# vaibhawvipul/taper

Hardware: AMD Instinct MI355X
Metric: MNIST samples/sec fwd+bwd+step (higher is better)
Workload: dtype f32; 1 GPU; mlp_784-128-10_b64; per_gpu_batch=64, global_batch=64, parallelism=single, comm=none, graph_record_steps=11577

## Files before the change

### include/taper_hip.h

```cpp
#ifndef TAPER_HIP_H
#define TAPER_HIP_H

#include <stddef.h>
#include <stdint.h>

#ifdef __cplusplus
extern "C" {
#endif

typedef struct th_ctx th_ctx;
typedef struct th_graph th_graph;
typedef struct th_event th_event;
typedef struct th_comm th_comm;

typedef struct th_adam_fuse {
    float *d_p, *d_m, *d_v;
    const int32_t *d_t;
    const float *d_lr;
    float beta1, beta2, eps, weight_decay;
} th_adam_fuse;

typedef struct th_adam_slice {
    const float *d_g;
    int64_t n;
// ... 68 lines not shown
                               int64_t *d_state, int64_t advance, int32_t *d_adam_tick, const th_adam_fuse *w_fuse,
                               const th_adam_fuse *b_fuse, int mask_dh_by_h);

int th_linear_xent_wide(th_ctx *ctx, const float *d_x, const float *d_w, const float *d_bias, const float *d_targets,
                        int batch, int in_features, int classes, float *d_loss, float *d_ncorrect,
                        float *d_dx, float *d_dw, float *d_db, float *d_metrics, int64_t metrics_capacity,
                        int64_t *d_state, int64_t advance, int32_t *d_adam_tick);
int th_linear_xent_wide_ex(th_ctx *ctx, const float *d_x, const float *d_w, const float *d_bias, const float *d_targets, int batch,
                           int in_features, int classes, float *d_loss, float *d_ncorrect, float *d_dx, float *d_dw, float *d_db,
                           float *d_metrics, int64_t metrics_capacity, int64_t *d_state, int64_t advance, int32_t *d_adam_tick,
                           float *d_colsum_masked);
int th_bias_from_colsum_adam(th_ctx *ctx, const float *d_colsum, float *d_gb, int c, int hw, const th_adam_fuse *b_fuse,
                             const th_adam_slice *extra, int n_extra);
typedef struct th_wide_fuse {
    th_adam_fuse w, b, conv_b;
    float *d_conv_gb;
    int conv_c, conv_hw;
} th_wide_fuse;
int th_linear_xent_wide_fused(th_ctx *ctx, const float *d_x, const float *d_w, const float *d_bias, const float *d_targets, int batch,
                              int in_features, int classes, float *d_loss, float *d_ncorrect, float *d_dw, float *d_db,
                              float *d_metrics, int64_t metrics_capacity, int64_t *d_state, int64_t advance, int32_t *d_adam_tick,
                              float *d_colsum_masked, const th_wide_fuse *fuse);

int th_mlp_tail_supported(int batch, int in_features, int hidden, int classes, int need_dx);
int th_mlp_tail(th_ctx *ctx, const float *d_x, const float *d_h, const float *d_w2, const float *d_b2,
                const float *d_targets, int batch, int in_features, int hidden, int classes,
                float *d_loss, float *d_ncorrect, float *d_dw1, float *d_db1, float *d_dw2, float *d_db2,
                const float *d_w1, float *d_dx,
                float *d_metrics, int64_t metrics_capacity, int64_t *d_state, int64_t advance,
                const th_adam_fuse *w1_fuse, const th_adam_fuse *b1_fuse);

typedef struct th_mlp3_layer {
    const float *d_w, *d_b;
    float *d_dw, *d_db;
    const th_adam_fuse *w_fuse, *b_fuse;
    int out_features;
} th_mlp3_layer;
typedef struct th_mlp3_gap {
    const float *d_cnt;
    float *d_gb;
    int hw;
    const th_adam_fuse *b_fuse;
} th_mlp3_gap;
int th_mlp3_supported(int batch, int in_features, int h1, int h2, int classes);
int th_mlp3_xent(th_ctx *ctx, const float *d_x, const float *d_targets, int batch, int in_features, const th_mlp3_layer *layers,
                 float *d_dx, float *d_loss, float *d_ncorrect, float *d_metrics, int64_t metrics_capacity, int64_t *d_state,
// ... 285 lines not shown
```

### taper_amd/csrc/host/modules.cpp

```cpp
#include <algorithm>
#include <chrono>
#include <cmath>
#include <cstdio>
#include <cstdlib>
#include <cstring>
#include <fstream>

#include "nn_internal.h"

namespace taper {
static float *n_correct_slot(Tensor *n_correct_out) {
    if (!n_correct_out) return nullptr;
    *n_correct_out = Tensor::empty({1});
    return n_correct_out->dptr();
}

static float *grad_slot(const Tensor &p) {
    if (!p.defined()) return nullptr;
    if (!p.grad_->buf) p.grad_->buf = Buffer::alloc(p.len());
    p.grad_->known_zero = false;
    return p.grad_->buf->d;
}

Tensor log_softmax(const Tensor &x, int dim) {
// ... 225 lines not shown
    TAPER_ASSERT(mlp_tail_supported(x, w1, b1, w2, b2), "mlp_tail_cross_entropy: unsupported shapes / gradient state");
    TAPER_ASSERT(targets.shape()[0] == x.shape()[0], "Batch sizes must match");
    const int b = (int)x.shape()[0], in_f = (int)x.shape()[1], hid = (int)w1.shape()[0], c = (int)w2.shape()[0];
    th_ctx *ctx = Device::ctx();
    Adam *fa = FusedAdamScope::active();
    th_adam_slice carried[TH_MAX_ADAM_SLICES];
    const int n_carried = fa ? fa->take_deferred(w1.dptr(), carried) : 0;
    if (fa && fa->has_deferred()) fa->flush_deferred();
    Tensor h = Tensor::empty({(size_t)b, (size_t)hid});
    TH(th_linear_fwd_ex(ctx, x.dptr(), w1.dptr(), b1.defined() ? b1.dptr() : nullptr, h.dptr(), b, in_f, hid, 1, carried, n_carried,
                        fa ? fa->d_tick() : nullptr));
    Tensor loss = Tensor::empty({1});
    float *nc = n_correct_slot(n_correct_out);
    float *dw1 = grad_slot(w1), *db1 = grad_slot(b1), *dw2 = grad_slot(w2), *db2 = grad_slot(b2);
    const bool need_dx = x.get_requires_grad();
    std::shared_ptr<Buffer> dx = need_dx ? Buffer::alloc(x.len()) : nullptr;
    th_adam_fuse wf{}, bf{};
    const th_adam_fuse *pw = nullptr, *pb = nullptr;
    if (fa) {
        if (!need_dx && fa->fuse_for(w1, &wf)) pw = &wf;
        if (b1.defined() && fa->fuse_for(b1, &bf)) pb = &bf;
    }
    const Communicator *xc = log ? log->exchange : nullptr;
    if (xc && xc->n_ranks > 1) {
        TAPER_ASSERT(fa && !need_dx && xc->tail_exchange_ok(b, in_f, hid, c), "mlp_tail_cross_entropy: the in-launch exchange does not cover this step");
        TH(th_mlp_tail_dp(xc->handle(), ctx, x.dptr(), h.dptr(), w2.dptr(), b2.defined() ? b2.dptr() : nullptr, targets.dptr(), b, in_f, hid, c,
                          loss.dptr(), nc, dw1, db1, dw2, db2, log ? log->d_metrics : nullptr, log ? log->capacity : 0,
                          log ? log->d_state : nullptr, log ? log->advance : 0, pw, pb, fa->d_tick()));
    } else
    TH(th_mlp_tail(ctx, x.dptr(), h.dptr(), w2.dptr(), b2.defined() ? b2.dptr() : nullptr, targets.dptr(), b, in_f, hid, c, loss.dptr(),
                   nc, dw1, db1, dw2, db2, need_dx ? w1.dptr() : nullptr, dx ? dx->d : nullptr, log ? log->d_metrics : nullptr,
                   log ? log->capacity : 0, log ? log->d_state : nullptr, log ? log->advance : 0, pw, pb));
    if (fa) {
        if (need_dx) fa->defer_for(w1);
        fa->defer_for(w2);
        if (b2.defined()) fa->defer_for(b2);
    }
    loss.set_requires_grad(true);
    Tensor p1 = w1, p2 = b1, p3 = w2, p4 = b2, out = loss, keep = h, xin = x;
    Tape::push(loss, true, [p1, p2, p3, p4, out, keep, xin, dx]() {
        if (!out.has_grad()) return;
        TAPER_ASSERT(out.grad_->shared_const, "mlp_tail_cross_entropy: only loss.backward() from the root is supported");
        if (dx) {
            TAPER_ASSERT(!xin.has_grad() && !xin.grad_->buf_is_arena, "mlp_tail_cross_entropy: input already has a gradient");
            xin.grad_->buf = dx;
            xin.grad_->has = true;
// ... 397 lines not shown
```

### taper_amd/csrc/host/taper.h

```cpp
#pragma once

#include <algorithm>
#include <cstdint>
#include <functional>
#include <map>
#include <memory>
#include <random>
#include <stdexcept>
#include <string>
#include <vector>

#include "../../../include/taper_hip.h"

namespace taper {

struct Error : std::runtime_error {
    explicit Error(const std::string &m) : std::runtime_error(m) {}
};
void th_check(int rc, const char *what);
#define TAPER_ASSERT(cond, msg)                       \
    do {                                              \
        if (!(cond)) throw ::taper::Error(msg);       \
    } while (0)

// ... 576 lines not shown
    bool step_reduced(const class Communicator &comm);
    void set_step_guard(const uint32_t *d_error_word) { step_guard_ = d_error_word; }
    void zero_grad() override { fp_.zero_grad(); }
    float get_lr() const { return lr_; }
    void set_lr(float lr);
    float weight_decay() const { return wd_; }
    float beta1() const { return beta1_; }
    float beta2() const { return beta2_; }
    float eps() const { return eps_; }
    void set_weight_decay(float wd) { wd_ = wd; }
    void load_state(int t, const std::vector<float> &m, const std::vector<float> &v);
    int t() const;
    std::vector<float> m() const;
    std::vector<float> v() const;
    FlatParams &flat() override { return fp_; }

    int32_t *d_tick() const { return reinterpret_cast<int32_t *>(state_->d); }
    bool fuse_for(const Tensor &param, th_adam_fuse *out);
    bool fuse_for_slot(const std::shared_ptr<GradSlot> &slot, th_adam_fuse *out);
    bool defer_for(const Tensor &param);
    int take_deferred(const float *launch_reads, th_adam_slice *out);
    void flush_deferred();
    void set_carry_deferred(bool on) { carry_deferred_ = on; }
    bool has_deferred() const { return !deferred_.empty(); }
    bool step_open() const { for (char f : fused_) if (f) return true; return !deferred_.empty(); }
    void set_external_tick(bool on) { external_tick_ = on; }
    void drop_step_bookkeeping() { deferred_.clear(); std::fill(fused_.begin(), fused_.end(), 0); }

   private:
    FlatParams fp_;
    std::shared_ptr<Buffer> m_, v_, state_;
    float lr_, beta1_, beta2_, eps_, wd_;
    bool external_tick_ = false;
    bool carry_deferred_ = false;
    const uint32_t *step_guard_ = nullptr;
    std::vector<char> fused_;
    std::vector<th_adam_slice> deferred_;
};

class AdamW : public Optimizer {
   public:
    AdamW(const std::vector<Tensor> &params, float lr, float beta1 = 0.9f, float beta2 = 0.999f, float eps = 1e-8f,
          float weight_decay = 0.0f)
        : adam(params, lr, beta1, beta2, eps, weight_decay) {}
    void step() override;
    void zero_grad() override { adam.zero_grad(); }
    FlatParams &flat() override { return adam.flat(); }
    float get_lr() const { return adam.get_lr(); }
    void set_lr(float lr) { adam.set_lr(lr); }
    Adam adam;
};

class LRScheduler {
   public:
    virtual ~LRScheduler() = default;
    virtual void step(const float *metric ) = 0;
    virtual float get_lr() const = 0;
// ... 226 lines not shown
```

### taper_amd/csrc/host/trainer.cpp

```cpp
#include <algorithm>
#include <chrono>
#include <cmath>
#include <cstdio>
#include <cstdlib>
#include <cstring>
#include <fstream>

#include "nn_internal.h"
#include "../../../include/taper_hip_debug.h"

namespace taper {
MNISTDataset MNISTDataset::from_host(const std::vector<float> &images, const std::vector<float> &labels, bool train) {
    TAPER_ASSERT(images.size() == labels.size() * 784, "MNISTDataset: images must be [N,784]");
    MNISTDataset d;
    d.images = Tensor(images, {labels.size(), 784});
    d.labels = Tensor(labels, {labels.size()});
    d.train = train;
    return d;
}

MNISTDataset MNISTDataset::from_u8(const std::vector<uint8_t> &pixels, const std::vector<uint8_t> &labels, bool train) {
    TAPER_ASSERT(pixels.size() == labels.size() * 784, "MNISTDataset: pixels must be [N,784]");
    th_ctx *ctx = Device::ctx();
    MNISTDataset d;
// ... 332 lines not shown
        case StepForm::Mlp2Rows: {
            std::vector<Tensor> w, b;
            for (Linear *l : plan.linear)
                if (l) {
                    w.push_back(l->weight);
                    b.push_back(l->bias);
                }
            loss = mlp2_cross_entropy(*rows, batch, w, b, &ncorrect, &sink);
            break;
        }
        case StepForm::ChainMlp3:
        case StepForm::Mlp3: {
            const Tensor w3[3] = {L[0]->weight, L[1]->weight, L[2]->weight}, b3[3] = {L[0]->bias, L[1]->bias, L[2]->bias};
            loss = plan.form == StepForm::ChainMlp3 ? conv_chain_mlp3_cross_entropy(xin, plan.stages, w3, b3, y, &ncorrect, &sink)
                                                    : mlp3_cross_entropy(seq->forward_prefix(xin, plan.prefix), w3, b3, y, &ncorrect, &sink);
            break;
        }
        case StepForm::ChainHead:
            loss = conv_chain_head_cross_entropy(xin, plan.stages, L[0]->weight, L[0]->bias, y, &ncorrect, &sink);
            break;
        case StepForm::MlpTail: {
            Tensor xh = seq->forward_prefix(xin, plan.prefix);
            if (plan.fused_adam) adam->set_carry_deferred(true);
            loss = mlp_tail_cross_entropy(xh, L[0]->weight, L[0]->bias, L[1]->weight, L[1]->bias, y, &ncorrect, &sink);
            break;
        }
        case StepForm::LinearHead:
        case StepForm::LinearWide: {
            adam->flush_deferred();
            Tensor h = seq->forward_prefix(xin, plan.prefix);
            loss = plan.form == StepForm::LinearHead ? linear_cross_entropy(h, L[0]->weight, L[0]->bias, y, &ncorrect, &sink)
                                                     : linear_cross_entropy_wide(h, L[0]->weight, L[0]->bias, y, &ncorrect, &sink);
            break;
        }
        case StepForm::Layered: {
            adam->flush_deferred();
            qat_pass_.run(*model);
            Tensor h = seq ? seq->forward_prefix(xin, plan.prefix) : model->forward(xin);
            for (size_t i = plan.prefix; seq && i < seq->layers.size(); ++i) h = seq->layers[i]->forward(h);
            loss = cross_entropy_loss(h, y, &ncorrect, &sink);
            break;
        }
    }
    loss.backward();
    if (plan.exchange) {
        optimizer->step();
    } else if (!(comm && optimizer->step_reduced(*comm))) {
        reduce_grads(*this);
        optimizer->step();
        optimizer->set_step_guard(nullptr);
    }
    optimizer->zero_grad();
    adam->set_carry_deferred(false);
}

void Trainer::enqueue_steps(const float *d_images, const float *d_labels, const int32_t *d_indices, int64_t n_indices,
                            size_t batch, size_t steps) {
    int64_t *state = reinterpret_cast<int64_t *>(state_->d);
    struct Guard {
        Guard(const uint32_t *w, uint32_t *step) { TH(th_ctx_set_update_guard(Device::ctx(), w, step)); }
        ~Guard() { th_ctx_set_update_guard(Device::ctx(), nullptr, nullptr); }
    } guard(comm && comm->is_p2p() ? comm->error_word() : nullptr, comm && comm->is_p2p() ? comm->step_word() : nullptr);
    TH(th_linear_fwd_ex_set_subtiles(Device::ctx(), !(comm && comm->ranks_on_this_device() > 1)));
    const StepPlan plan = plan_step(batch, d_indices ? n_indices : (int64_t)batch);
    if (plan.form == StepForm::Mlp2Rows) {
        const th_row_source rows{d_images, d_labels, d_indices, d_indices ? state + 1 : nullptr, d_indices ? n_indices : 0,
                                 d_indices ? n_indices : (int64_t)batch};
        for (size_t s = 0; s < steps; ++s) enqueue_compute(plan, nullptr, nullptr, batch, &rows);
    } else if (d_indices == nullptr) {
        enqueue_compute(plan, const_cast<float *>(d_images), const_cast<float *>(d_labels), batch);
    } else {
        TH(th_gather_batch(Device::ctx(), d_images, d_labels, d_indices, n_indices, state + 1, (int)(batch * steps), 784, xb_->d,
                           yb_->d));
        for (size_t s = 0; s < steps; ++s) enqueue_compute(plan, xb_->d + s * batch * 784, yb_->d + s * batch, batch);
    }
    optimizer->flush_deferred();
// ... 135 lines not shown
        }
        std::sort(graphs_.begin(), graphs_.end(), [](const auto &x, const auto &y) { return x.first > y.first; });
        graph_key_ = key;
    }
    if (!whole) {
        const size_t tail = n_full - done > 0 ? (n_full - done) % chunk : 0;
        size_t exact = 0;
        for (auto &g : graphs_) exact += (g.first & (g.first - 1)) != 0 ? 1 : 0;
        if (tail > 2 && (tail & (tail - 1)) != 0 && !have(tail) && have(1) && exact < 4 && !graph_capture_failed_ &&
            graph_key_ == key) {
            TH(th_graph_begin(ctx));
            th_graph *g = nullptr;
            try {
                enqueue_steps(d_img, d_lab, d_idx, (int64_t)n, bs, tail);
                TH(th_graph_end(ctx, &g));
                graphs_.emplace_back(tail, g);
                std::sort(graphs_.begin(), graphs_.end(), [](const auto &x, const auto &y) { return x.first > y.first; });
            } catch (const std::exception &e) {
                fprintf(stderr, "taper: capturing a %zu-step remainder graph failed (%s); the ladder graphs serve it\n", tail, e.what());
                if (!g) th_graph_end(ctx, &g);
                if (g) th_graph_destroy(g);
                if (auto *adam = dynamic_cast<Adam *>(optimizer.get())) {
                    adam->set_carry_deferred(false);
                    adam->drop_step_bookkeeping();
                }
                optimizer->zero_grad();
                Tape::reset();
                if (!comm) throw;
            }
        }
    }
    if (!whole && done == 0 && nb == n_full && n_full >= 2 && have(n_full) && whole_graphs_.size() < 4 && !graph_capture_failed_ && graph_key_ == key &&
        std::find(whole_capture_failed_.begin(), whole_capture_failed_.end(), n_full) == whole_capture_failed_.end()) {
        TH(th_graph_begin(ctx));
        th_graph *g = nullptr;
        try {
            TH(th_fill_f32(ctx, state_->d, 0.f, 4));
            enqueue_steps(d_img, d_lab, d_idx, (int64_t)n, bs, n_full);
            TH(th_graph_end(ctx, &g));
            whole_graphs_.emplace_back(n_full, g);
            TH(th_graph_launch(ctx, g));
            done = n_full;
        } catch (const std::exception &e) {
            fprintf(stderr, "taper: capturing a whole-call graph of %zu steps failed (%s); reset + replay stay two launches\n", n_full, e.what());
            whole_capture_failed_.push_back(n_full);
            if (!g) th_graph_end(ctx, &g);
            if (g) th_graph_destroy(g);
            if (auto *adam = dynamic_cast<Adam *>(optimizer.get())) {
                adam->set_carry_deferred(false);
                adam->drop_step_bookkeeping();
            }
            optimizer->zero_grad();
            Tape::reset();
            if (!comm) throw;
        }
    }
    while (done < n_full) {
        bool launched = false;
        for (auto &g : graphs_) {
            if (done + g.first <= n_full) {
                TH(th_graph_launch(ctx, g.second));
                done += g.first;
                launched = true;
                break;
            }
        }
        if (!launched) {
            enqueue_steps(d_img, d_lab, d_idx, (int64_t)n, bs, 1);
            ++done;
        }
    }
    if (nb > n_full) {
// ... 32 lines not shown
```

### taper_amd/csrc/mlp_tail.hip

```cpp
#include "tail_dev.h"
#include "dp_dev.h"

TH_USES_DEVICE_ERRORS()

namespace th {

struct TailArgs {
    const float *x, *h, *w2, *b2, *targets;
    int batch, in_f, hid, c;
    float *loss, *ncorrect, *dw1, *db1, *dw2, *db2;
    float *metrics;
    int64_t capacity;
    int64_t *state;
    int64_t advance;
    AdamDev w1_adam, b1_adam;
    int n_dw, n_head, tiles_m, groups;
    const float *w1;
    float *dx;
    int xgroups;
    DpDev dp;
    int32_t *dp_tick;
};

#ifdef TH_PROFILE
// ... 416 lines not shown
    int64_t log_slot = 0, state0_next = 0, state1_next = 0;
    if (log) {
        const int64_t state0 = sload(a.state), state1 = sload(a.state + 1);
        log_slot = tail_log_slot(state0, a.capacity);
        state0_next = state0 + 1;
        state1_next = state1 + a.advance;
    }
    if (lane == 0) *h_step = step;
    __syncthreads();
    if (lead) {
        if (a.db2 && lane < a.c) {
            float sum = sc[0][16 + lane];
#pragma unroll
            for (int w = 1; w < NW; ++w) sum += sc[w][16 + lane];
            a.db2[lane] = sum;
        }
        if (lane == 0) tail_lead_log<NW>(a, sc, log_slot, state0_next, state1_next);
#ifdef TH_PROFILE
        if (lane == 0) tail_prof_end(wall_clock64());
#endif
    }
}

template <int KS, int TN, bool HAS_DX, int NW, int DPNR = 0>
__global__ __launch_bounds__(64 * (NW + tail_helper_waves(KS, NW, DPNR))) void mlp_tail_exact_kernel(TailArgs a) {
    constexpr unsigned HID = 16 * KS;
    constexpr bool HELPER = tail_helper_waves(KS, NW, DPNR) != 0;
    __shared__ float h_step;
    __shared__ float red[NW][TN][64][4];
    __shared__ float tr[NW][16][17];
    __shared__ float rowv[NW][2][16];
    __shared__ float sc[NW][36];
    asm volatile("" ::"s"(a.x), "s"(a.h), "s"(a.w2), "s"(a.b2), "s"(a.targets), "s"(a.batch), "s"(a.in_f), "s"(a.c), "s"(a.dw1),
                 "s"(a.db1), "s"(a.w1_adam.p), "s"(a.w1_adam.m), "s"(a.w1_adam.v), "s"(a.w1_adam.t), "s"(a.w1_adam.lr),
                 "s"(a.b1_adam.p), "s"(a.b1_adam.t), "s"(a.b1_adam.lr), "s"(a.n_dw), "s"(a.n_head), "s"(a.groups), "s"(a.metrics),
                 "s"(a.state));
    const int t = threadIdx.x, lane = t & 63, wave = t >> 6, r16 = lane & 15, g4 = lane >> 4;
    const int bid = blockIdx.x;
    TAIL_STAMP(0);
    DpTicket dp_tk{0u, 0u};
    if constexpr (DPNR > 0) dp_tk = dp_begin(a.dp);
    if (HAS_DX && bid >= a.n_head + a.n_dw) {
        if (!HELPER || wave < NW) tail_dx_role<KS, NW>(a, bid - a.n_head - a.n_dw);
        return;
    }
    const bool head_role = bid < a.n_head;
    int tile_m, grp = 0, tt = 0;
    if (!head_role) {
        const int b2 = bid - a.n_head;
        tt = (b2 & 7) * (a.n_dw >> 3) + (b2 >> 3);
        if (tt >= KS * a.groups) return;
        tile_m = tt % KS;
        grp = tt / KS;
    } else {
// ... 9 lines not shown
    if constexpr (HELPER) {
        if (__builtin_amdgcn_readfirstlane(wave) == NW) {
            tail_helper_wave<NW>(a, head_role, lead, any_w, any_b, &h_step, sc);
            return;
        }
    }
    const int32_t w_t = (!HELPER && any_w) ? sload(a.w1_adam.t) : 1, b_t = (!HELPER && any_b) ? sload(a.b1_adam.t) : 1;
    const float w_lr = (!HELPER && any_w) ? sload(a.w1_adam.lr) : 0.f, b_lr = (!HELPER && any_b) ? sload(a.b1_adam.lr) : 0.f;

    float4 wv[KS];
    const unsigned w_off = ((unsigned)min(r16, C - 1) * HID + g4 * 4) * 4u;
#pragma unroll
    for (int ks = 0; ks < KS; ++ks) wv[ks] = ldg4_b(a.w2, w_off + ks * 64);
    float w2b[4], b2v[4];
#pragma unroll
    for (int s = 0; s < 4; ++s) {
        const unsigned cls = (unsigned)min(g4 * 4 + s, C - 1);
        w2b[s] = ldg_b(a.w2, (cls * HID + hcol) * 4u);
        b2v[s] = a.b2 ? ldg_b(a.b2, cls * 4u) : 0.f;
    }
    bool tn_ok[TN];
#pragma unroll
    for (int tn = 0; tn < TN; ++tn) tn_ok[tn] = col0 + tn * 16 < in_f;
    const unsigned e_off = ((tile_m * 16 + g4 * 4 + wave) * in_f + col0 + r16) * 4u;
    const bool fuse_w = !head_role && any_w;
    const bool finisher = NW == 4 || wave < 4;
    float e_p[TN], e_m[TN], e_v[TN], w_step = 0.f, b_step = 0.f;
#pragma unroll
    for (int tn = 0; tn < TN; ++tn) {
        e_p[tn] = e_m[tn] = e_v[tn] = 0.f;
        if (fuse_w && tn_ok[tn] && finisher) {
            e_p[tn] = ldg_b(a.w1_adam.p, e_off + tn * 64);
            e_m[tn] = ldg_b(a.w1_adam.m, e_off + tn * 64);
            e_v[tn] = ldg_b(a.w1_adam.v, e_off + tn * 64);
        }
    }
    const bool fuse_b1 = head_role && any_b;
    const unsigned b1_off = (tile_m * 16 + (t & 15)) * 4u;
    float bp_ = 0.f, bm_ = 0.f, bv_ = 0.f;
    if (fuse_b1) {
        bp_ = ldg_b(a.b1_adam.p, b1_off);
        bm_ = ldg_b(a.b1_adam.m, b1_off);
        bv_ = ldg_b(a.b1_adam.v, b1_off);
    }
    const bool log_here = !HELPER && lead && a.metrics;
    const int64_t state0 = log_here ? sload(a.state) : 0, state1 = log_here ? sload(a.state + 1) : 0;

    floatx4 accdw[TN];
#pragma unroll
    for (int tn = 0; tn < TN; ++tn) accdw[tn] = floatx4{0.f, 0.f, 0.f, 0.f};
    floatx4 acc_dw2 = {0.f, 0.f, 0.f, 0.f};
    float db1_acc = 0.f, db2_acc = 0.f, nll_acc = 0.f, hit_acc = 0.f;
    const float inv_b = 1.0f / (float)B;

    float4 hv[KS];
    float tf = 0.f, hm[4], xv[TN][4];
    auto load_chunk = [&](int c0) {
        const int r0 = c0 + wave * 16;
        if (r0 >= B) return;
        const unsigned h_off = ((unsigned)(r0 + r16) * HID + g4 * 4) * 4u;
#pragma unroll
        for (int ks = 0; ks < KS; ++ks) hv[ks] = ldg4_b(a.h, h_off + ks * 64);
        tf = ldg_b(a.targets, (unsigned)(r0 + r16) * 4u);
        const unsigned hm_off = ((unsigned)(r0 + g4 * 4) * HID + hcol) * 4u;
        const unsigned x_off = ((unsigned)(r0 + g4 * 4) * in_f + col0 + r16) * 4u;
#pragma unroll
        for (int s = 0; s < 4; ++s) {
            hm[s] = ldg_b(a.h, hm_off + s * HID * 4);
#pragma unroll
            for (int tn = 0; tn < TN; ++tn)
                xv[tn][s] = (!head_role && tn_ok[tn]) ? ldg_b(a.x, x_off + s * in_f * 4u + tn * 64) : 0.f;
        }
    };
    load_chunk(0);
    TAIL_STAMP(1);
    if (!HELPER && fuse_w) w_step = adam_step_size(w_lr, a.w1_adam.beta1, a.w1_adam.beta2, w_t);
    if (!HELPER && fuse_b1) b_step = adam_step_size(b_lr, a.b1_adam.beta1, a.b1_adam.beta2, b_t);
    int64_t log_slot = 0, state0_next = 0, state1_next = 0;
    if (log_here) {
        log_slot = tail_log_slot(state0, a.capacity);
        state0_next = state0 + 1;
        state1_next = state1 + a.advance;
    }
    TAIL_STAMP(2);

    for (int c0 = 0;;) {
        const int r0 = c0 + wave * 16;
        const bool rows_here = r0 < B;
        if (rows_here) {
            TAIL_STAMP(3);
            floatx4 ax = {0.f, 0.f, 0.f, 0.f}, ay = ax, az = ax, aw = ax;
#pragma unroll
            for (int ks = 0; ks < KS; ++ks) {
                ax = __builtin_amdgcn_mfma_f32_16x16x4f32(wv[ks].x, hv[ks].x, ax, 0, 0, 0);
// ... 7 lines not shown
            for (int i = 0; i < 4; ++i) lg[i] = (g4 * 4 + i < C) ? ((ax[i] + ay[i]) + (az[i] + aw[i])) + b2v[i] : -INFINITY;
            tail_row_softmax(lg, g4, C, tf, inv_b, dl, nll_row, bi);
            TAIL_STAMP(4);

            floatx4 dh = {0.f, 0.f, 0.f, 0.f};
#pragma unroll
            for (int s = 0; s < 4; ++s) dh = __builtin_amdgcn_mfma_f32_16x16x4f32(dl[s], w2b[s], dh, 0, 0, 0);
            float dhm[4];
#pragma unroll
            for (int i = 0; i < 4; ++i) dhm[i] = hm[i] > 0.f ? dh[i] : 0.f;

            if (!head_role) {
#pragma unroll
                for (int s = 0; s < 4; ++s)
#pragma unroll
                    for (int tn = 0; tn < TN; ++tn)
                        accdw[tn] = __builtin_amdgcn_mfma_f32_16x16x4f32(dhm[s], xv[tn][s], accdw[tn], 0, 0, 0);
            } else {
                db1_acc += sum_over_g4((dhm[0] + dhm[1]) + (dhm[2] + dhm[3]));
                __builtin_amdgcn_wave_barrier();
#pragma unroll
                for (int i = 0; i < 4; ++i) tr[wave][r16][g4 * 4 + i] = dl[i];
                if (lead && g4 == 0) {
                    rowv[wave][0][r16] = nll_row;
                    rowv[wave][1][r16] = (fabsf((float)bi - tf) < 1e-6f) ? 1.f : 0.f;
                }
                __builtin_amdgcn_wave_barrier();
#pragma unroll
                for (int s = 0; s < 4; ++s)
                    acc_dw2 = __builtin_amdgcn_mfma_f32_16x16x4f32(tr[wave][g4 * 4 + s][r16], hm[s], acc_dw2, 0, 0, 0);
                if (lead) {
                    float cs = 0.f, nl = 0.f, ht = 0.f;
#pragma unroll
                    for (int r = 0; r < 16; ++r) {
                        cs += tr[wave][r][r16];
                        nl += rowv[wave][0][r];
                        ht += rowv[wave][1][r];
                    }
                    db2_acc += cs;
                    nll_acc += nl;
                    hit_acc += ht;
                }
            }
        }
        c0 += 16 * NW;
        if (c0 >= B) break;
        load_chunk(c0);
    }

    TAIL_STAMP(5);
    if (!head_role) {
#pragma unroll
        for (int tn = 0; tn < TN; ++tn)
#pragma unroll
            for (int i = 0; i < 4; ++i) red[wave][tn][lane][i] = accdw[tn][i];
        __syncthreads();
        TAIL_STAMP(6);
        if (HELPER && fuse_w) w_step = h_step;
        float outv[TN];
#pragma unroll
        for (int tn = 0; tn < TN; ++tn) {
            outv[tn] = 0.f;
            if (!tn_ok[tn] || !finisher) continue;
            float out = red[0][tn][lane][wave];
#pragma unroll
            for (int w = 1; w < NW; ++w) out += red[w][tn][lane][wave];
            outv[tn] = out;
        }
        if constexpr (DPNR > 0) {
            if (!dp_reduce<DPNR, TN>(a.dp, dp_tk, KS + tt, finisher ? t : -1, outv)) return;
        }
#pragma unroll
        for (int tn = 0; tn < TN; ++tn) {
            if (!tn_ok[tn] || !finisher) continue;
            const float out = outv[tn];
            if (DPNR == 0 || !fuse_w) *reinterpret_cast<float *>(reinterpret_cast<char *>(a.dw1) + e_off + tn * 64) = out;
            if (fuse_w) {
                const AdamDev &ad = a.w1_adam;
                const float gv = out + ad.wd * e_p[tn];
                const float mn = ad.beta1 * e_m[tn] + (1.0f - ad.beta1) * gv;
                const float vn = ad.beta2 * e_v[tn] + (1.0f - ad.beta2) * gv * gv;
                *reinterpret_cast<float *>(reinterpret_cast<char *>(ad.m) + e_off + tn * 64) = mn;
                *reinterpret_cast<float *>(reinterpret_cast<char *>(ad.v) + e_off + tn * 64) = vn;
                *reinterpret_cast<float *>(reinterpret_cast<char *>(ad.p) + e_off + tn * 64) = e_p[tn] - w_step * mn / (sqrtf(vn) + ad.eps);
            }
        }
        TAIL_STAMP(7);
        return;
    }

#pragma unroll
    for (int i = 0; i < 4; ++i) red[wave][0][lane][i] = acc_dw2[i];
    if (g4 == 0) sc[wave][r16] = db1_acc;
    if (lead && g4 == 0) sc[wave][16 + r16] = db2_acc;
    if (lead && lane == 0) {
        sc[wave][32] = nll_acc;
        sc[wave][33] = hit_acc;
    }
    __syncthreads();
    TAIL_STAMP(6);
    if (HELPER && fuse_b1) b_step = h_step;
    if constexpr (DPNR > 0) {
        float hv2[2] = {0.f, 0.f};
        const int cls = g4 * 4 + wave;
        if (a.dw2 && wave < 4 && cls < C) {
            float sum = red[0][0][lane][wave];
#pragma unroll
            for (int w = 1; w < NW; ++w) sum += red[w][0][lane][wave];
            hv2[0] = sum;
        }
        if (a.db1 && t < 16) {
            float out = sc[0][t];
#pragma unroll
            for (int w = 1; w < NW; ++w) out += sc[w][t];
            hv2[1] = out;
        } else if (lead && a.db2 && t >= 16 && t < 16 + C) {
            float sum = sc[0][t];
#pragma unroll
// ... 61 lines not shown
            }
            const float l = n / (float)B;
            a.loss[0] = l;
            if (a.ncorrect) a.ncorrect[0] = hsum;
            if (a.metrics) {
                a.metrics[2 * log_slot] = l;
                a.metrics[2 * log_slot + 1] = hsum;
                a.state[0] = state0_next;
                a.state[1] = state1_next;
            }
        }
    }
    TAIL_STAMP(7);
}

}

using namespace th;

static bool tail_whole_tiles(int batch, int in_features, int hidden) {
    return (hidden == 32 || hidden == 64 || hidden == 128 || hidden == 256) && batch % 16 == 0 && in_features % 16 == 0;
}

extern "C" int th_mlp_tail_supported(int batch, int in_features, int hidden, int classes, int need_dx) {
    const bool ok = batch > 0 && batch <= 512 && in_features > 0 && hidden > 0 && hidden <= 256 && (hidden % 4) == 0 && classes > 0 &&
                    classes <= 16;
    return ok && (!need_dx || tail_whole_tiles(batch, in_features, hidden));
}

static bool tail_dp_shapes(int batch, int in_features, int hidden, int classes) {
    return th_mlp_tail_supported(batch, in_features, hidden, classes, 0) && tail_whole_tiles(batch, in_features, hidden) &&
           (hidden == 64 || hidden == 128);
}
static int tail_dp_grid(int in_features, int hidden) {
    const int tiles_m = hidden / 16, groups = ceil_div(in_features, 32);
    return ((tiles_m * groups + 7) & ~7) + ((tiles_m + 7) & ~7);
}
template <int KS, int NW>
static const void *tail_dp_instance(int n_ranks) {
    if (n_ranks <= 2) return (const void *)mlp_tail_exact_kernel<KS, 2, false, NW, 2>;
    if (n_ranks <= 4) return (const void *)mlp_tail_exact_kernel<KS, 2, false, NW, 4>;
    return (const void *)mlp_tail_exact_kernel<KS, 2, false, NW, 8>;
}
static int tail_exact_threads(int ks, int nw, bool dp) { return 64 * (nw + tail_helper_waves(ks, nw, dp ? 2 : 0)); }
static const void *tail_dp_kernel(int batch, int hidden, int n_ranks) {
    const bool nw8 = batch > 64;
// ... 2 lines not shown
}

extern "C" int th_mlp_tail_dp_supported(const th_comm *comm, th_ctx *ctx, int batch, int in_features, int hidden, int classes) {
    const DpDev *dp = comm_dp_dev(comm);
    if (!dp || !ctx || dp->n_ranks < 2 || !tail_dp_shapes(batch, in_features, hidden, classes)) return 0;
    const int grid = tail_dp_grid(in_features, hidden);
    if (grid > DP_MAX_SLOTS) return 0;
    if (comm_dp_sharing(comm) > 1) {
        int per_cu = 0;
        if (hipOccupancyMaxActiveBlocksPerMultiprocessor(&per_cu, tail_dp_kernel(batch, hidden, dp->n_ranks), tail_exact_threads(hidden / 16, batch > 64 ? 8 : 4, true), 0) != hipSuccess) {
            (void)hipGetLastError();
            return 0;
        }
        if (!comm_dp_shared_fits(comm, grid, per_cu)) return 0;
    }
    return 1;
}

static int mlp_tail_launch(th_comm *comm, th_ctx *ctx, const float *d_x, const float *d_h, const float *d_w2, const float *d_b2,
                           const float *d_targets, int batch, int in_features, int hidden, int classes, float *d_loss,
                           float *d_ncorrect, float *d_dw1, float *d_db1, float *d_dw2, float *d_db2, const float *d_w1, float *d_dx,
                           float *d_metrics, int64_t metrics_capacity, int64_t *d_state, int64_t advance,
                           const th_adam_fuse *w1_fuse, const th_adam_fuse *b1_fuse, int32_t *d_tick) {
    TH_REQUIRE(ctx && d_x && d_h && d_w2 && d_targets && d_loss && d_dw1, "th_mlp_tail: null argument");
    TH_REQUIRE(th_mlp_tail_supported(batch, in_features, hidden, classes, 0),
               "th_mlp_tail: needs batch <= 512, hidden <= 256 and a multiple of 4, classes <= 16 (got %d, %d, %d)", batch, hidden, classes);
    TH_REQUIRE(!d_dx || (d_w1 && tail_whole_tiles(batch, in_features, hidden)),
               "th_mlp_tail: d_dx needs d_w1 and whole tiles (hidden 32 / 64 / 128 / 256, batch and in_features multiples of 16)");
    TH_REQUIRE(!d_dx || !(w1_fuse && w1_fuse->d_p), "th_mlp_tail: with d_dx the launch reads W1, its update must be deferred (th_adam_slice)");
    TH_REQUIRE((((uintptr_t)d_h | (uintptr_t)d_w2) & 15) == 0, "th_mlp_tail: d_h and d_w2 must be 16-byte aligned");
    TH_REQUIRE(!d_metrics || (d_state && metrics_capacity > 0), "th_mlp_tail: metrics need d_state and a capacity");
    TH_REQUIRE(!(b1_fuse && b1_fuse->d_p) || d_db1, "th_mlp_tail: fused b1 update needs d_db1");
    constexpr int TN = 2;
    TailArgs a{};
    a.x = d_x; a.h = d_h; a.w2 = d_w2; a.b2 = d_b2; a.targets = d_targets;
    a.batch = batch; a.in_f = in_features; a.hid = hidden; a.c = classes;
    a.loss = d_loss; a.ncorrect = d_ncorrect; a.dw1 = d_dw1; a.db1 = d_db1; a.dw2 = d_dw2; a.db2 = d_db2;
    a.metrics = d_metrics; a.capacity = metrics_capacity; a.state = d_state; a.advance = advance;
    a.w1_adam = make_adam_dev(w1_fuse);
    a.b1_adam = make_adam_dev(b1_fuse);
    a.tiles_m = ceil_div(hidden, 16);
    a.groups = ceil_div(in_features, 16 * TN);
    a.n_dw = (a.tiles_m * a.groups + 7) & ~7;
    a.n_head = (a.tiles_m + 7) & ~7;
    a.w1 = d_w1;
    a.dx = d_dx;
    a.xgroups = ceil_div(in_features, 32);
    const int nw = batch <= 64 ? 4 : 8;
    const int grid = a.n_dw + a.n_head + (d_dx ? a.xgroups * ceil_div(batch, 16 * nw) : 0);
    const bool exact = tail_whole_tiles(batch, in_features, hidden);
    if (comm) {
        const DpDev *dp = comm_dp_dev(comm);
        TH_REQUIRE(dp && th_mlp_tail_dp_supported(comm, ctx, batch, in_features, hidden, classes),
                   "th_mlp_tail_dp: this communicator / shape cannot take the in-launch exchange (th_mlp_tail_dp_supported)");
        TH_REQUIRE(!d_dx && exact && grid == tail_dp_grid(in_features, hidden), "th_mlp_tail_dp: internal: launch shape");
        a.dp = *dp;
        a.dp_tick = d_tick;
        const void *fn = tail_dp_kernel(batch, hidden, dp->n_ranks);
        void *args[] = {&a};
        TH_HIP(hipLaunchKernel(fn, dim3(grid), dim3(tail_exact_threads(hidden / 16, nw, true)), args, 0, ctx->stream));
        comm_dp_count_launch(comm);
        return 0;
    }
#define TH_TAIL_LAUNCH(KS)                                                                                            \
    do {                                                                                                              \
        if (exact && d_dx && nw == 8) hipLaunchKernelGGL((mlp_tail_exact_kernel<KS, TN, true, 8>), dim3(grid), dim3(512), 0, ctx->stream, a);     \
        else if (exact && d_dx) hipLaunchKernelGGL((mlp_tail_exact_kernel<KS, TN, true, 4>), dim3(grid), dim3(tail_exact_threads(KS, 4, false)), 0, ctx->stream, a);     \
        else if (exact && nw == 8) hipLaunchKernelGGL((mlp_tail_exact_kernel<KS, TN, false, 8>), dim3(grid), dim3(512), 0, ctx->stream, a);     \
        else if (exact) hipLaunchKernelGGL((mlp_tail_exact_kernel<KS, TN, false, 4>), dim3(grid), dim3(tail_exact_threads(KS, 4, false)), 0, ctx->stream, a);     \
        else hipLaunchKernelGGL((mlp_tail_kernel<KS, TN>), dim3(grid), dim3(256), 0, ctx->stream, a);                 \
    } while (0)
    if (exact && hidden == 32) TH_TAIL_LAUNCH(2);
    else if (hidden <= 64) TH_TAIL_LAUNCH(4);
    else if (hidden <= 128) TH_TAIL_LAUNCH(8);
    else TH_TAIL_LAUNCH(16);
#undef TH_TAIL_LAUNCH
    TH_LAUNCH_CHECK();
    return 0;
}

extern "C" int th_mlp_tail(th_ctx *ctx, const float *d_x, const float *d_h, const float *d_w2, const float *d_b2,
                           const float *d_targets, int batch, int in_features, int hidden, int classes, float *d_loss,
                           float *d_ncorrect, float *d_dw1, float *d_db1, float *d_dw2, float *d_db2, const float *d_w1, float *d_dx,
                           float *d_metrics, int64_t metrics_capacity, int64_t *d_state, int64_t advance,
                           const th_adam_fuse *w1_fuse, const th_adam_fuse *b1_fuse) {
    return mlp_tail_launch(nullptr, ctx, d_x, d_h, d_w2, d_b2, d_targets, batch, in_features, hidden, classes, d_loss, d_ncorrect, d_dw1, d_db1,
                           d_dw2, d_db2, d_w1, d_dx, d_metrics, metrics_capacity, d_state, advance, w1_fuse, b1_fuse, nullptr);
}

// ... 27 lines not shown
```

### taper_amd/csrc/tail_dev.h

```cpp
#pragma once
#include "adam_dev.h"

namespace th {

typedef float floatx4 __attribute__((ext_vector_type(4)));

__device__ __forceinline__ float ldg_b(const float *base, unsigned byte_off) {
    return *reinterpret_cast<const float *>(reinterpret_cast<const char *>(base) + byte_off);
}
__device__ __forceinline__ float4 ldg4_b(const float *base, unsigned byte_off) {
    return *reinterpret_cast<const float4 *>(reinterpret_cast<const char *>(base) + byte_off);
}
__device__ __forceinline__ void pair16(float x, float &lo, float &hi) {
    const auto r = __builtin_amdgcn_permlane16_swap(__float_as_uint(x), __float_as_uint(x), false, false);
    lo = __uint_as_float(r[0]);
    hi = __uint_as_float(r[1]);
}
__device__ __forceinline__ void pair32(float x, float &lo, float &hi) {
    const auto r = __builtin_amdgcn_permlane32_swap(__float_as_uint(x), __float_as_uint(x), false, false);
    lo = __uint_as_float(r[0]);
    hi = __uint_as_float(r[1]);
}
__device__ __forceinline__ float sum_over_g4(float x) {
    float lo, hi;
    pair16(x, lo, hi);
    x = lo + hi;
    pair32(x, lo, hi);
    return lo + hi;
}
__device__ __forceinline__ void argmax_step(float &best, int &bi, float v0, float v1, float i0, float i1) {
    const int j0 = __float_as_int(i0), j1 = __float_as_int(i1);
// ... 47 lines not shown
```

Measured before the change: 5.679 million samples/s.

## Skip dense dW1 write when Adam is fused and vectorize tail kernel column pairs

When Adam is fused into the MLP tail on a single GPU with whole tiles, the host now passes a null dW1 pointer, so the kernel no longer writes the dense first-layer gradient to memory. A new 'wide' kernel variant has each lane handle two adjacent columns and uses float2 loads and stores for x, the weight, the Adam moments and dW1. It also simplifies the lead-wave reductions for db2, nll and hits through a padded shared-memory layout. The cost is extra template instantiations, alignment checks, and dW1 being unavailable to any consumer outside the fused step.

After: 5.238 million samples/s. -7.8%, worse.

```diff
diff --git a/include/taper_hip.h b/include/taper_hip.h
--- a/include/taper_hip.h
+++ b/include/taper_hip.h
@@ -114,6 +114,7 @@
                               float *d_metrics, int64_t metrics_capacity, int64_t *d_state, int64_t advance, int32_t *d_adam_tick,
                               float *d_colsum_masked, const th_wide_fuse *fuse);
 
+int th_mlp_tail_dw1_optional(int batch, int in_features, int hidden);
 int th_mlp_tail_supported(int batch, int in_features, int hidden, int classes, int need_dx);
 int th_mlp_tail(th_ctx *ctx, const float *d_x, const float *d_h, const float *d_w2, const float *d_b2,
                 const float *d_targets, int batch, int in_features, int hidden, int classes,
diff --git a/taper_amd/csrc/host/modules.cpp b/taper_amd/csrc/host/modules.cpp
--- a/taper_amd/csrc/host/modules.cpp
+++ b/taper_amd/csrc/host/modules.cpp
@@ -271,6 +271,7 @@
         if (b1.defined() && fa->fuse_for(b1, &bf)) pb = &bf;
     }
     const Communicator *xc = log ? log->exchange : nullptr;
+    if (pw && fa->drop_fused_grads() && !(xc && xc->n_ranks > 1) && th_mlp_tail_dw1_optional(b, in_f, hid)) dw1 = nullptr;
     if (xc && xc->n_ranks > 1) {
         TAPER_ASSERT(fa && !need_dx && xc->tail_exchange_ok(b, in_f, hid, c), "mlp_tail_cross_entropy: the in-launch exchange does not cover this step");
         TH(th_mlp_tail_dp(xc->handle(), ctx, x.dptr(), h.dptr(), w2.dptr(), b2.defined() ? b2.dptr() : nullptr, targets.dptr(), b, in_f, hid, c,
diff --git a/taper_amd/csrc/host/taper.h b/taper_amd/csrc/host/taper.h
--- a/taper_amd/csrc/host/taper.h
+++ b/taper_amd/csrc/host/taper.h
@@ -622,6 +622,8 @@
     int take_deferred(const float *launch_reads, th_adam_slice *out);
     void flush_deferred();
     void set_carry_deferred(bool on) { carry_deferred_ = on; }
+    void set_drop_fused_grads(bool on) { drop_fused_grads_ = on; }
+    bool drop_fused_grads() const { return drop_fused_grads_; }
     bool has_deferred() const { return !deferred_.empty(); }
     bool step_open() const { for (char f : fused_) if (f) return true; return !deferred_.empty(); }
     void set_external_tick(bool on) { external_tick_ = on; }
@@ -633,6 +635,7 @@
     float lr_, beta1_, beta2_, eps_, wd_;
     bool external_tick_ = false;
     bool carry_deferred_ = false;
+    bool drop_fused_grads_ = false;
     const uint32_t *step_guard_ = nullptr;
     std::vector<char> fused_;
     std::vector<th_adam_slice> deferred_;
diff --git a/taper_amd/csrc/host/trainer.cpp b/taper_amd/csrc/host/trainer.cpp
--- a/taper_amd/csrc/host/trainer.cpp
+++ b/taper_amd/csrc/host/trainer.cpp
@@ -378,6 +378,7 @@
         case StepForm::MlpTail: {
             Tensor xh = seq->forward_prefix(xin, plan.prefix);
             if (plan.fused_adam) adam->set_carry_deferred(true);
+            if (plan.fused_adam && !comm) adam->set_drop_fused_grads(true);
             loss = mlp_tail_cross_entropy(xh, L[0]->weight, L[0]->bias, L[1]->weight, L[1]->bias, y, &ncorrect, &sink);
             break;
         }
@@ -408,6 +409,7 @@
     }
     optimizer->zero_grad();
     adam->set_carry_deferred(false);
+    adam->set_drop_fused_grads(false);
 }
 
 void Trainer::enqueue_steps(const float *d_images, const float *d_labels, const int32_t *d_indices, int64_t n_indices,
@@ -589,6 +591,7 @@
                 if (g) th_graph_destroy(g);
                 if (auto *adam = dynamic_cast<Adam *>(optimizer.get())) {
                     adam->set_carry_deferred(false);
+                    adam->set_drop_fused_grads(false);
                     adam->drop_step_bookkeeping();
                 }
                 optimizer->zero_grad();
@@ -615,6 +618,7 @@
             if (g) th_graph_destroy(g);
             if (auto *adam = dynamic_cast<Adam *>(optimizer.get())) {
                 adam->set_carry_deferred(false);
+                adam->set_drop_fused_grads(false);
                 adam->drop_step_bookkeeping();
             }
             optimizer->zero_grad();
diff --git a/taper_amd/csrc/mlp_tail.hip b/taper_amd/csrc/mlp_tail.hip
--- a/taper_amd/csrc/mlp_tail.hip
+++ b/taper_amd/csrc/mlp_tail.hip
@@ -462,14 +462,17 @@
     }
 }
 
-template <int KS, int TN, bool HAS_DX, int NW, int DPNR = 0>
+template <int KS, int TN, bool HAS_DX, int NW, int DPNR = 0, bool WIDE = false>
 __global__ __launch_bounds__(64 * (NW + tail_helper_waves(KS, NW, DPNR))) void mlp_tail_exact_kernel(TailArgs a) {
+    static_assert(!WIDE || (TN == 2 && DPNR == 0), "the wide form: two adjacent columns per lane, single GPU");
     constexpr unsigned HID = 16 * KS;
     constexpr bool HELPER = tail_helper_waves(KS, NW, DPNR) != 0;
+    constexpr bool LEAD1 = DPNR == 0;
+    constexpr int RS = LEAD1 ? 17 : 1;
     __shared__ float h_step;
     __shared__ float red[NW][TN][64][4];
     __shared__ float tr[NW][16][17];
-    __shared__ float rowv[NW][2][16];
+    __shared__ float rowv[NW][2][16 * RS];
     __shared__ float sc[NW][36];
     asm volatile("" ::"s"(a.x), "s"(a.h), "s"(a.w2), "s"(a.b2), "s"(a.targets), "s"(a.batch), "s"(a.in_f), "s"(a.c), "s"(a.dw1),
                  "s"(a.db1), "s"(a.w1_adam.p), "s"(a.w1_adam.m), "s"(a.w1_adam.v), "s"(a.w1_adam.t), "s"(a.w1_adam.lr),
@@ -525,17 +528,27 @@
     bool tn_ok[TN];
 #pragma unroll
     for (int tn = 0; tn < TN; ++tn) tn_ok[tn] = col0 + tn * 16 < in_f;
-    const unsigned e_off = ((tile_m * 16 + g4 * 4 + wave) * in_f + col0 + r16) * 4u;
+    const bool pair_ok = col0 + 2 * r16 < in_f;
+    const unsigned cpair = min(col0 + 2 * r16, in_f - 2);
+    const unsigned e_off = WIDE ? ((tile_m * 16 + g4 * 4 + wave) * in_f + cpair) * 4u : ((tile_m * 16 + g4 * 4 + wave) * in_f + col0 + r16) * 4u;
     const bool fuse_w = !head_role && any_w;
     const bool finisher = NW == 4 || wave < 4;
     float e_p[TN], e_m[TN], e_v[TN], w_step = 0.f, b_step = 0.f;
-#pragma unroll
-    for (int tn = 0; tn < TN; ++tn) {
-        e_p[tn] = e_m[tn] = e_v[tn] = 0.f;
-        if (fuse_w && tn_ok[tn] && finisher) {
-            e_p[tn] = ldg_b(a.w1_adam.p, e_off + tn * 64);
-            e_m[tn] = ldg_b(a.w1_adam.m, e_off + tn * 64);
-            e_v[tn] = ldg_b(a.w1_adam.v, e_off + tn * 64);
+    if constexpr (WIDE) {
+        e_p[0] = e_p[1] = e_m[0] = e_m[1] = e_v[0] = e_v[1] = 0.f;
+        if (fuse_w && finisher) {
+            const float2 p2 = ldg2_b(a.w1_adam.p, e_off), m2 = ldg2_b(a.w1_adam.m, e_off), v2 = ldg2_b(a.w1_adam.v, e_off);
+            e_p[0] = p2.x, e_p[1] = p2.y, e_m[0] = m2.x, e_m[1] = m2.y, e_v[0] = v2.x, e_v[1] = v2.y;
+        }
+    } else {
+#pragma unroll
+        for (int tn = 0; tn < TN; ++tn) {
+            e_p[tn] = e_m[tn] = e_v[tn] = 0.f;
+            if (fuse_w && tn_ok[tn] && finisher) {
+                e_p[tn] = ldg_b(a.w1_adam.p, e_off + tn * 64);
+                e_m[tn] = ldg_b(a.w1_adam.m, e_off + tn * 64);
+                e_v[tn] = ldg_b(a.w1_adam.v, e_off + tn * 64);
+            }
         }
     }
     const bool fuse_b1 = head_role && any_b;
@@ -566,13 +579,18 @@
         for (int ks = 0; ks < KS; ++ks) hv[ks] = ldg4_b(a.h, h_off + ks * 64);
         tf = ldg_b(a.targets, (unsigned)(r0 + r16) * 4u);
         const unsigned hm_off = ((unsigned)(r0 + g4 * 4) * HID + hcol) * 4u;
-        const unsigned x_off = ((unsigned)(r0 + g4 * 4) * in_f + col0 + r16) * 4u;
+        const unsigned x_off = WIDE ? ((unsigned)(r0 + g4 * 4) * in_f + cpair) * 4u : ((unsigned)(r0 + g4 * 4) * in_f + col0 + r16) * 4u;
 #pragma unroll
         for (int s = 0; s < 4; ++s) {
             hm[s] = ldg_b(a.h, hm_off + s * HID * 4);
-#pragma unroll
-            for (int tn = 0; tn < TN; ++tn)
-                xv[tn][s] = (!head_role && tn_ok[tn]) ? ldg_b(a.x, x_off + s * in_f * 4u + tn * 64) : 0.f;
+            if constexpr (WIDE) {
+                const float2 x2 = !head_role ? ldg2_b(a.x, x_off + s * in_f * 4u) : make_float2(0.f, 0.f);
+                xv[0][s] = x2.x, xv[TN - 1][s] = x2.y;
+            } else {
+#pragma unroll
+                for (int tn = 0; tn < TN; ++tn)
+                    xv[tn][s] = (!head_role && tn_ok[tn]) ? ldg_b(a.x, x_off + s * in_f * 4u + tn * 64) : 0.f;
+            }
         }
     };
     load_chunk(0);
@@ -626,14 +644,20 @@
 #pragma unroll
                 for (int i = 0; i < 4; ++i) tr[wave][r16][g4 * 4 + i] = dl[i];
                 if (lead && g4 == 0) {
-                    rowv[wave][0][r16] = nll_row;
-                    rowv[wave][1][r16] = (fabsf((float)bi - tf) < 1e-6f) ? 1.f : 0.f;
+                    rowv[wave][0][r16 * RS] = nll_row;
+                    rowv[wave][1][r16 * RS] = (fabsf((float)bi - tf) < 1e-6f) ? 1.f : 0.f;
                 }
                 __builtin_amdgcn_wave_barrier();
 #pragma unroll
                 for (int s = 0; s < 4; ++s)
                     acc_dw2 = __builtin_amdgcn_mfma_f32_16x16x4f32(tr[wave][g4 * 4 + s][r16], hm[s], acc_dw2, 0, 0, 0);
-                if (lead) {
+                if (lead && LEAD1) {
+                    const float *src = g4 == 0 ? &tr[wave][0][r16] : &rowv[wave][g4 == 2 ? 1 : 0][0];
+                    float sum = 0.f;
+#pragma unroll
+                    for (int r = 0; r < 16; ++r) sum += src[r * 17];
+                    db2_acc += sum;
+                } else if (lead) {
                     float cs = 0.f, nl = 0.f, ht = 0.f;
 #pragma unroll
                     for (int r = 0; r < 16; ++r) {
@@ -665,7 +689,7 @@
 #pragma unroll
         for (int tn = 0; tn < TN; ++tn) {
             outv[tn] = 0.f;
-            if (!tn_ok[tn] || !finisher) continue;
+            if (!(WIDE ? pair_ok : tn_ok[tn]) || !finisher) continue;
             float out = red[0][tn][lane][wave];
 #pragma unroll
             for (int w = 1; w < NW; ++w) out += red[w][tn][lane][wave];
@@ -673,12 +697,33 @@
         }
         if constexpr (DPNR > 0) {
             if (!dp_reduce<DPNR, TN>(a.dp, dp_tk, KS + tt, finisher ? t : -1, outv)) return;
+        }
+        if constexpr (WIDE) {
+            if (pair_ok && finisher) {
+                if (a.dw1) stg2_b(a.dw1, e_off, outv[0], outv[1]);
+                if (fuse_w) {
+                    const AdamDev &ad = a.w1_adam;
+                    float mn[2], vn[2], pn[2];
+#pragma unroll
+                    for (int tn = 0; tn < 2; ++tn) {
+                        const float gv = outv[tn] + ad.wd * e_p[tn];
+                        mn[tn] = ad.beta1 * e_m[tn] + (1.0f - ad.beta1) * gv;
+                        vn[tn] = ad.beta2 * e_v[tn] + (1.0f - ad.beta2) * gv * gv;
+                        pn[tn] = e_p[tn] - w_step * mn[tn] / (sqrtf(vn[tn]) + ad.eps);
+                    }
+                    stg2_b(ad.m, e_off, mn[0], mn[1]);
+                    stg2_b(ad.v, e_off, vn[0], vn[1]);
+                    stg2_b(ad.p, e_off, pn[0], pn[1]);
+                }
+            }
+            TAIL_STAMP(7);
+            return;
         }
 #pragma unroll
         for (int tn = 0; tn < TN; ++tn) {
             if (!tn_ok[tn] || !finisher) continue;
             const float out = outv[tn];
-            if (DPNR == 0 || !fuse_w) *reinterpret_cast<float *>(reinterpret_cast<char *>(a.dw1) + e_off + tn * 64) = out;
+            if (DPNR == 0 ? a.dw1 != nullptr : !fuse_w) *reinterpret_cast<float *>(reinterpret_cast<char *>(a.dw1) + e_off + tn * 64) = out;
             if (fuse_w) {
                 const AdamDev &ad = a.w1_adam;
                 const float gv = out + ad.wd * e_p[tn];
@@ -697,7 +742,9 @@
     for (int i = 0; i < 4; ++i) red[wave][0][lane][i] = acc_dw2[i];
     if (g4 == 0) sc[wave][r16] = db1_acc;
     if (lead && g4 == 0) sc[wave][16 + r16] = db2_acc;
-    if (lead && lane == 0) {
+    if constexpr (LEAD1) {
+        if (lead && (lane == 16 || lane == 32)) sc[wave][32 + (lane >> 5)] = db2_acc;
+    } else if (lead && lane == 0) {
         sc[wave][32] = nll_acc;
         sc[wave][33] = hit_acc;
     }
@@ -805,6 +852,8 @@
     return (hidden == 32 || hidden == 64 || hidden == 128 || hidden == 256) && batch % 16 == 0 && in_features % 16 == 0;
 }
 
+extern "C" int th_mlp_tail_dw1_optional(int batch, int in_features, int hidden) { return tail_whole_tiles(batch, in_features, hidden) ? 1 : 0; }
+
 extern "C" int th_mlp_tail_supported(int batch, int in_features, int hidden, int classes, int need_dx) {
     const bool ok = batch > 0 && batch <= 512 && in_features > 0 && hidden > 0 && hidden <= 256 && (hidden % 4) == 0 && classes > 0 &&
                     classes <= 16;
@@ -853,7 +902,9 @@
                            float *d_ncorrect, float *d_dw1, float *d_db1, float *d_dw2, float *d_db2, const float *d_w1, float *d_dx,
                            float *d_metrics, int64_t metrics_capacity, int64_t *d_state, int64_t advance,
                            const th_adam_fuse *w1_fuse, const th_adam_fuse *b1_fuse, int32_t *d_tick) {
-    TH_REQUIRE(ctx && d_x && d_h && d_w2 && d_targets && d_loss && d_dw1, "th_mlp_tail: null argument");
+    TH_REQUIRE(ctx && d_x && d_h && d_w2 && d_targets && d_loss, "th_mlp_tail: null argument");
+    TH_REQUIRE(d_dw1 || (!comm && w1_fuse && w1_fuse->d_p && tail_whole_tiles(batch, in_features, hidden)),
+               "th_mlp_tail: d_dw1 may be null only with w1_fuse, on one GPU, for whole tiles (th_mlp_tail_dw1_optional)");
     TH_REQUIRE(th_mlp_tail_supported(batch, in_features, hidden, classes, 0),
                "th_mlp_tail: needs batch <= 512, hidden <= 256 and a multiple of 4, classes <= 16 (got %d, %d, %d)", batch, hidden, classes);
     TH_REQUIRE(!d_dx || (d_w1 && tail_whole_tiles(batch, in_features, hidden)),
@@ -880,6 +931,9 @@
     const int nw = batch <= 64 ? 4 : 8;
     const int grid = a.n_dw + a.n_head + (d_dx ? a.xgroups * ceil_div(batch, 16 * nw) : 0);
     const bool exact = tail_whole_tiles(batch, in_features, hidden);
+    uintptr_t wide_bits = (uintptr_t)d_x | (uintptr_t)d_dw1;
+    if (w1_fuse && w1_fuse->d_p) wide_bits |= (uintptr_t)w1_fuse->d_p | (uintptr_t)w1_fuse->d_m | (uintptr_t)w1_fuse->d_v;
+    const bool wide = exact && !comm && (wide_bits & 7) == 0;
     if (comm) {
         const DpDev *dp = comm_dp_dev(comm);
         TH_REQUIRE(dp && th_mlp_tail_dp_supported(comm, ctx, batch, in_features, hidden, classes),
@@ -895,7 +949,11 @@
     }
 #define TH_TAIL_LAUNCH(KS)                                                                                            \
     do {                                                                                                              \
-        if (exact && d_dx && nw == 8) hipLaunchKernelGGL((mlp_tail_exact_kernel<KS, TN, true, 8>), dim3(grid), dim3(512), 0, ctx->stream, a);     \
+        if (wide && d_dx && nw == 8) hipLaunchKernelGGL((mlp_tail_exact_kernel<KS, TN, true, 8, 0, true>), dim3(grid), dim3(512), 0, ctx->stream, a);     \
+        else if (wide && d_dx) hipLaunchKernelGGL((mlp_tail_exact_kernel<KS, TN, true, 4, 0, true>), dim3(grid), dim3(tail_exact_threads(KS, 4, false)), 0, ctx->stream, a);     \
+        else if (wide && nw == 8) hipLaunchKernelGGL((mlp_tail_exact_kernel<KS, TN, false, 8, 0, true>), dim3(grid), dim3(512), 0, ctx->stream, a);     \
+        else if (wide) hipLaunchKernelGGL((mlp_tail_exact_kernel<KS, TN, false, 4, 0, true>), dim3(grid), dim3(tail_exact_threads(KS, 4, false)), 0, ctx->stream, a);     \
+        else if (exact && d_dx && nw == 8) hipLaunchKernelGGL((mlp_tail_exact_kernel<KS, TN, true, 8>), dim3(grid), dim3(512), 0, ctx->stream, a);     \
         else if (exact && d_dx) hipLaunchKernelGGL((mlp_tail_exact_kernel<KS, TN, true, 4>), dim3(grid), dim3(tail_exact_threads(KS, 4, false)), 0, ctx->stream, a);     \
         else if (exact && nw == 8) hipLaunchKernelGGL((mlp_tail_exact_kernel<KS, TN, false, 8>), dim3(grid), dim3(512), 0, ctx->stream, a);     \
         else if (exact) hipLaunchKernelGGL((mlp_tail_exact_kernel<KS, TN, false, 4>), dim3(grid), dim3(tail_exact_threads(KS, 4, false)), 0, ctx->stream, a);     \
diff --git a/taper_amd/csrc/tail_dev.h b/taper_amd/csrc/tail_dev.h
--- a/taper_amd/csrc/tail_dev.h
+++ b/taper_amd/csrc/tail_dev.h
@@ -7,6 +7,12 @@
 
 __device__ __forceinline__ float ldg_b(const float *base, unsigned byte_off) {
     return *reinterpret_cast<const float *>(reinterpret_cast<const char *>(base) + byte_off);
+}
+__device__ __forceinline__ float2 ldg2_b(const float *base, unsigned byte_off) {
+    return *reinterpret_cast<const float2 *>(reinterpret_cast<const char *>(base) + byte_off);
+}
+__device__ __forceinline__ void stg2_b(float *base, unsigned byte_off, float x, float y) {
+    *reinterpret_cast<float2 *>(reinterpret_cast<char *>(base) + byte_off) = make_float2(x, y);
 }
 __device__ __forceinline__ float4 ldg4_b(const float *base, unsigned byte_off) {
     return *reinterpret_cast<const float4 *>(reinterpret_cast<const char *>(base) + byte_off);
```
